# Jerx2y/Raytracer-2022

Measured on AMD Instinct MI355X. Metric: Mrays/s (primary+secondary), book-2 final scene 800x800x1000spp, higher is better.
Workload: dtype f64

## Files before the change

raytracer_2022_amd/csrc/hip/pt_device.h:

```cpp
#ifndef RT2022_PT_DEVICE_H
#define RT2022_PT_DEVICE_H

#include <hip/hip_runtime.h>
#include <stdint.h>

#include <vector>

#include "../../../include/rt2022.h"
#include "hip_owned.hpp"

namespace rt2022 {

struct MediumDev {
    double center[3], radius;
    double neg_inv_density;
    uint32_t boundary, mat;
    uint32_t sphere_boundary;
    uint32_t _pad[3];
};

struct MaterialDev {
    uint32_t tex, tex_kind;
    double albedo[3];
    double param;
// ... 27 lines not shown
    const MediumDev *media_dev;
    uint32_t media_mode;
    uint32_t n_nodes;
    uint32_t n_xforms, n_media;
    uint32_t n_spheres, n_moving_spheres;
    uint32_t n_rects;
};

struct StatsDev {
    unsigned long long paths, rays, node_visits;
    unsigned long long prim_tests[RT_KIND_COUNT];
    unsigned long long light_pdf_tests, rng_draws;
    unsigned long long op_rounds[9], op_lanes[9];
};

struct RenderArgs {
    rt_camera cam;
    uint32_t width, height, spp, max_depth;
    uint32_t n_frames, n_rows;
    uint32_t chunk, n_chunks;
    double background[3];
    double t_min;
    uint64_t seed;
    uint64_t n_pixels;
    uint64_t n_items;
    const uint32_t *row_ids;
    double *partial;
    unsigned long long *work_counter;
    double *tape;
    uint32_t ring, ring_group;
    const unsigned long long *claim_limit;
    uint32_t tuning;
    uint32_t vote_weights;
    StatsDev *stats;
    const rt_radiance_ray *rays;
};

enum SlotKind : uint32_t {
    SK_IDLE = 0,
    SK_FRESH = 1,
    SK_TRACE = 2,
    SK_MISS = 3,
    SK_LIGHT = 4,
    SK_LAMB_SOLID = 5,
    SK_LAMB_CHECKER = 6,
    SK_LAMB_NOISE = 7,
    SK_LAMB_IMAGE = 8,
    SK_METAL = 9,
    SK_DIELECTRIC = 10,
    SK_ISOTROPIC = 11,
    SK_COUNT = 12
};

constexpr uint32_t kMatKindShift = 24, kMatIndexMask = (1u << kMatKindShift) - 1u;

constexpr int kSlotsPerBlock = 4096;
constexpr uint64_t kRecBytes = 128, kRecDoubles = kRecBytes / 8, kRecWords = kRecBytes / 4;
struct WfPool {
    uint32_t n_slots;
    uint32_t n_blocks;
    uint8_t *kind;
    double *ray;
    uint32_t *hit;
    uint32_t *state;
    double *pixel_sum;
    double *tape;
    uint32_t tape_cap;
    uint16_t *list;
    uint32_t *list_n;
    uint32_t segs;
    uint32_t *next_chunk;
    uint32_t *max_list;
    uint32_t n_cus;
    uint32_t *n_active;
    uint32_t *fault;
    unsigned long long *oldest;
    uint32_t *starved_n;
    unsigned long long *dbg;
};

namespace tune {
constexpr uint32_t kSegmentsShift = 16, kClassShift = 20, kGroupsShift = 24;
constexpr uint32_t kNoNodeTable = 1u << 28, kPassTiming = 1u << 29, kLiteralStep = 1u << 30, kBoxesPlain = 1u << 31;
constexpr uint32_t quorum(uint32_t word) { return word & 0xFFu; }
constexpr uint32_t segments(uint32_t word) { return (word >> kSegmentsShift) & 0xFu; }
constexpr uint32_t class_shift(uint32_t word) { return (word >> kClassShift) & 0xFu; }
constexpr uint32_t groups(uint32_t word) { return (word >> kGroupsShift) & 0xFu; }
constexpr bool no_node_table(uint32_t word) { return (word & kNoNodeTable) != 0; }
constexpr bool pass_timing(uint32_t word) { return (word & kPassTiming) != 0; }
constexpr bool literal_step(uint32_t word) { return (word & kLiteralStep) != 0; }
constexpr bool boxes_plain(uint32_t word) { return (word >> 31) != 0; }
constexpr uint32_t for_kernels(uint32_t word, bool plain) { return (word & ~kBoxesPlain) | (plain && !literal_step(word) ? kBoxesPlain : 0u); }
constexpr uint32_t kRetiredDefault = (1u << 8) | (2u << 12);
constexpr uint32_t kDefault = 18u | kRetiredDefault | ((uint32_t)(8 * 4096 / kSlotsPerBlock > 0 ? 8 * 4096 / kSlotsPerBlock : 1) << kSegmentsShift) |
                              (2u << kClassShift) | (0u << kGroupsShift);
static_assert(kDefault == 0x00282112u, "the default tuning word");
}

constexpr int kStackSmall = 22;
constexpr int kStackMid = 30;
constexpr int kStackLarge = 64;
constexpr int kBlock = 256;
constexpr uint32_t kWfVoteWeights = 0x24444442u;
constexpr int kCacheBlock = 1024;
constexpr int kStackTiny = 16;
constexpr int kNodeCache = 1740;
constexpr int kPrimNodes = 600, kPrimSpheres = 256, kPrimMoving = 512;
constexpr int kTraceBlocksPerCU = 4;

struct QueryArgs {
    const rt_query_ray *rays;
    rt_hit *hits;
    uint64_t n_rays;
    unsigned long long *counter;
    StatsDev *stats;
};
hipError_t launch_query(const SceneDev &scene, const QueryArgs &args, uint32_t stack_need, bool counters, bool any_hit,
                        hipStream_t stream);

struct FeatureArgs {
    rt_camera cam;
    uint32_t width, height, spp, n_rows;
    double background[3];
    double t_min;
    uint64_t seed;
    uint64_t n_pixels;
    const uint32_t *row_ids;
    rt_feature *out;
    unsigned long long *counter;
    StatsDev *stats;
};
hipError_t launch_features(const SceneDev &scene, const FeatureArgs &args, uint32_t stack_need, bool counters, hipStream_t stream);

hipError_t launch_render(const SceneDev &scene, const RenderArgs &args, uint32_t stack_need, bool counters,
                         int n_blocks_hint, hipStream_t stream);
constexpr unsigned kFeatMisc = 1;
constexpr unsigned kFeatMovers = 2;
constexpr unsigned kFeatVolumes = 4;

constexpr int kMaxGroups = 8;
// ... 59 lines not shown
```

raytracer_2022_amd/csrc/hip/pt_wavefront.hip:

```cpp
#include <algorithm>
#include <cstdio>
#include <cstdlib>
#include <type_traits>
#include <vector>

#include "pt_common.hpp"

namespace rt2022 {

namespace {

constexpr int S = kSlotsPerBlock;
constexpr uint32_t kOriginClasses = 4u;
constexpr uint32_t kListBins = 16 * kOriginClasses * 8;
constexpr uint32_t kChunk = 256;
constexpr int kShadeWaves = 3;
constexpr int kLeanBlocks = 5;
constexpr int kSphereReps = 2, kNodeReps = 1, kBoxReps = 2, kMiscReps = 2;

typedef double f64x2 __attribute__((ext_vector_type(2)));
typedef double f64x2_a8 __attribute__((ext_vector_type(2), aligned(8)));
typedef uint32_t u32x4 __attribute__((ext_vector_type(4)));
typedef uint32_t u32x2 __attribute__((ext_vector_type(2)));
typedef float f32x2 __attribute__((ext_vector_type(2)));
// ... 139 lines not shown
        }
        case RT_KIND_RECT: {
            RectP rp{(uint32_t)rtm::d2u(q.r2.y), q.r0.x, q.r0.y, q.r1.x, q.r1.y, q.r2.x};
            rect_record(rp, 0u, r, t, rec);
            break;
        }
        case RT_KIND_BOX: {
            const double p0x = q.r0.x, p0y = q.r0.y, p0z = q.r1.x, p1x = q.r1.y, p1y = q.r2.x, p1z = q.r2.y;
            const uint32_t i = w.face;
            RectP rp;
            if (i < 2) rp = RectP{RT_RECT_XY, p0x, p1x, p0y, p1y, i == 0 ? p1z : p0z};
            else if (i < 4) rp = RectP{RT_RECT_XZ, p0x, p1x, p0z, p1z, i == 2 ? p1y : p0y};
            else rp = RectP{RT_RECT_YZ, p0y, p1y, p0z, p1z, i == 4 ? p1x : p0x};
            rect_record(rp, 0u, r, t, rec);
            break;
        }
        case RT_KIND_TRIANGLE: {
            const Vec3 a(q.r0.x, q.r0.y, q.r1.x), b(q.r1.y, q.r2.x, q.r2.y), c(q.r3.x, q.r3.y, q.r4.x);
            Vec3 n = rtm::to_unit(rtm::cross(b - a, c - a));
            Vec3 p = r.o + r.d * t;
            double a1 = a.x - b.x, b1 = a.x - c.x, c1 = a.x - p.x;
            double a2 = a.y - b.y, b2 = a.y - c.y, c2 = a.y - p.y;
            rec.u = (c1 * b2 - b1 * c2) / (a1 * b2 - b1 * a2);
            rec.v = (a1 * c2 - a2 * c1) / (a1 * b2 - b1 * a2);
            rec.p = p; rec.t = t;
            rec.set_face_normal(r.d, n);
            break;
        }
        case RT_KIND_RING: {
            rec.p = r.o + r.d * t; rec.t = t; rec.u = 0.0; rec.v = 0.0;
            rec.set_face_normal(r.d, Vec3(0.0, 1.0, 0.0));
            break;
        }
        default: {
            rec.p = r.o + r.d * t; rec.normal = Vec3(1.0, 0.0, 0.0); rec.t = t; rec.u = 0.0; rec.v = 0.0;
            rec.front_face = true;
            break;
        }
    }
    if (w.leaf & RT_REF_FLIP) rec.front_face = !rec.front_face;
    for (uint32_t lvl = w.chain.n; lvl > 0; lvl--) {
        XRay moved = ray_at_level(s, w.chain, lvl, world);
        xform_record(s, w.chain.at(lvl - 1), moved, rec);
    }
}
RT_DEV Vec3 texture_value_top(const SceneDev &s, uint32_t tex, uint32_t tex_kind, Vec3 color, double u, double v, Vec3 p) {
    if (tex_kind == RT_TEX_SOLID) return color;
    return texture_value(s, tex, u, v, p);
}

}

#ifdef RT2022_SHADE_PROBE
#define SP_DECL unsigned long long sp_t = wall_clock64(), sp_acc[10] = {0, 0, 0, 0, 0, 0, 0, 0, 0, 0}
#define SP_MARK(i) do { unsigned long long sp_n = wall_clock64(); sp_acc[i] += sp_n - sp_t; sp_t = sp_n; } while (0)
#define SP_FLUSH() do { if (tid == 0 && pool.dbg) for (int sp_i = 0; sp_i < 10; sp_i++) atomicAdd(&pool.dbg[64 + sp_i], sp_acc[sp_i]); } while (0)
#else
#define SP_DECL do {} while (0)
#define SP_MARK(i) do {} while (0)
#define SP_FLUSH() do {} while (0)
#endif

template <bool STATS, bool RING = false, bool RAYS = false>
__global__ void __launch_bounds__(kBlock, kShadeWaves) wf_shade(const SceneDev s, const RenderArgs *__restrict__ ap, const WfPool pool, const uint32_t parity) {
    __shared__ uint32_t hist[SK_COUNT];
    __shared__ uint32_t cursor[SK_COUNT];
    __shared__ uint32_t sorted[S];
    __shared__ uint32_t n_sorted;
    __shared__ uint8_t new_kind[S];
    __shared__ uint32_t bins[kListBins];
    __shared__ uint8_t new_oct[S];
    __shared__ uint16_t fresh_q[S];
    static_assert(kSlotsPerBlock <= 32768 && kSlotsPerBlock % kBlock == 0, "a segment's slot index shares a u16 with one flag bit (fresh_q), and the sorts deal S / kBlock slots to every thread");
    static_assert(kSlotsPerBlock <= 65536, "`sorted` packs slot | kind << 16");
    __shared__ uint32_t n_fresh;
    const RenderArgs &a = *ap;
    const PoolView pv{pool};
    const uint32_t base = blockIdx.x * (uint32_t)S;
    const uint32_t tid = threadIdx.x;
    const unsigned lane = tid & 63u;
    Counters<STATS> cnt;

    constexpr uint32_t kLdsLights = 8;
    __shared__ LightRec lights_lds[kLdsLights];
    __shared__ PrimTable prim_tab;
    prim_table_fill(s, prim_tab, tid);
    if (tid < kLdsLights && tid < s.n_lights) lights_lds[tid] = fetch_light(s, tid);
    auto light_at = [&](uint32_t li) { return li < kLdsLights ? lights_lds[li] : fetch_light(s, li); };
    SP_DECL;
    if (tid < SK_COUNT) hist[tid] = 0;
    if (tid == 0) n_fresh = 0;
    __syncthreads();
    const uint32_t n_rays = pool.list_n[blockIdx.x] < (uint32_t)S ? pool.list_n[blockIdx.x] : (uint32_t)S;
    const uint32_t n_starved_in = RING ? (pool.starved_n[blockIdx.x] < (uint32_t)S - n_rays ? pool.starved_n[blockIdx.x] : (uint32_t)S - n_rays) : 0u;
    const uint32_t n_listed = n_rays + n_starved_in;
    uint32_t my_kind[S / kBlock], my_slot[S / kBlock];
#pragma unroll
    for (int i = 0; i < S / kBlock; i++) {
        const uint32_t e = (uint32_t)(i * kBlock) + tid;
        uint32_t k = SK_IDLE, ls = 0;
        if (e < n_listed) { k = pool.kind[base + e]; ls = pool.list[base + e]; }
        my_kind[i] = k; my_slot[i] = ls;
        new_kind[e] = (uint8_t)SK_IDLE;
        if (k != SK_IDLE) atomicAdd(&hist[k], 1u);
    }
    __syncthreads();
    if (tid == 0) {
        uint32_t acc = 0;
        for (uint32_t k = 0; k < SK_COUNT; k++) { cursor[k] = acc; acc += hist[k]; }
        n_sorted = acc;
    }
    __syncthreads();
#pragma unroll
    for (int i = 0; i < S / kBlock; i++) {
        uint32_t k = my_kind[i];
        if (k != SK_IDLE) sorted[atomicAdd(&cursor[k], 1u)] = my_slot[i] | (k << 16);
    }
    __syncthreads();
    SP_MARK(0);
    const uint32_t total = n_sorted;
    const Vec3 background = ld3(a.background);
    const bool single = a.chunk == 1 && a.spp > 0 && a.max_depth > 0;
    const bool small_job = a.n_items <= 0xFFFFFFFFull;
    const uint32_t step_shift = tune::class_shift(a.tuning);

    unsigned long long my_oldest = ~0ull;
    for (uint32_t j0 = 0; j0 < total; j0 += kBlock) {
        const uint32_t j = j0 + tid;
        const bool on = j < total;
        uint32_t slot = 0, kind = SK_IDLE;
        if (on) { uint32_t e = sorted[j]; slot = base + (e & 0xFFFFu); kind = e >> 16; }
        if (on && kind == SK_TRACE) atomicOr(pool.fault, 1u);
        bool alive = false;
        bool ended = false;
        Ray r;
        Rng rng;
        Vec3 Lterm(0.0, 0.0, 0.0);
        SlotTape tape{pool.tape + (uint64_t)slot * pool.tape_cap * 4};
        SlotState stt{};
        Winner w;
        w.t = 0.0; w.leaf = 0; w.face = 0; w.chain.n = 0; w.chain.c0 = w.chain.c1 = w.chain.c2 = w.chain.c3 = 0;
        uint32_t steps = 0;
        uint32_t mat_word = 0;
        PrimRegs prim{{0.0, 0.0}, {0.0, 0.0}, {0.0, 0.0}, {0.0, 0.0}, {0.0, 0.0}};
        f64x2 md0{0.0, 0.0}, md1{0.0, 0.0}, md2{0.0, 0.0}, md3{0.0, 0.0}, md4{0.0, 0.0};
        if (on) {
            stt = load_state(pool, slot);
            if (kind > SK_MISS) {
                uint64_t rs;
                r = pv.load_ray(slot, rs);
                rng = Rng(rs);
                const u32x4 *hq = reinterpret_cast<const u32x4 *>(pool.hit + (uint64_t)slot * kRecWords);
                u32x4 ha = hq[0], hb = hq[1];
                t_pin(ha); t_pin(hb);
                bool have_mat;
                PoolView::decode_hit(ha, hb, w, steps, mat_word, have_mat);
                if (!have_mat) mat_word = leaf_material_word(s, w.leaf);
                const f64x2_a8 *pp = prim_address(prim_tab, w.leaf);
                const f64x2 *mp = reinterpret_cast<const f64x2 *>(s.materials_dev + (mat_word & kMatIndexMask));
                prim.r0 = pp[0]; prim.r1 = pp[1]; prim.r2 = pp[2]; prim.r3 = pp[3]; prim.r4 = pp[4];
                md0 = mp[0]; md1 = mp[1]; md2 = mp[2]; md3 = mp[3]; md4 = mp[4];
                t_pin(prim.r0); t_pin(prim.r1); t_pin(prim.r2); t_pin(prim.r3); t_pin(prim.r4);
                t_pin(md0); t_pin(md1); t_pin(md2); t_pin(md3); t_pin(md4);
            }
        }
        SP_MARK(1);
        const uint32_t m_tex = (uint32_t)rtm::d2u(md0.x), m_tex_kind = (uint32_t)(rtm::d2u(md0.x) >> 32);
        const Vec3 m_albedo(md0.y, md1.x, md1.y), m_tex_color(md2.y, md3.x, md3.y);
        const double m_param = md2.x;
        uint32_t depth = stt.depth & 0x7FFFFFFFu;
        uint32_t tainted = stt.depth >> 31;
        uint32_t expect = steps;

        if (on && kind >= SK_MISS) {
            if (kind == SK_MISS) {
                Lterm = background;
                ended = true;
            } else {
                bool want_uv = false;
                const bool lambertian = kind >= SK_LAMB_SOLID && kind <= SK_LAMB_IMAGE;
                if (lambertian) {
                    want_uv = kind == SK_LAMB_IMAGE || kind == SK_LAMB_CHECKER;
                } else if (kind == SK_LIGHT || kind == SK_ISOTROPIC) {
                    want_uv = m_tex_kind == RT_TEX_IMAGE || m_tex_kind == RT_TEX_CHECKER;
                }
                HitRec rec;
                winner_record_regs(s, r, w, prim, rec, want_uv);
                SP_MARK(2);
                if (kind == SK_LIGHT) {
                    Lterm = rec.front_face ? texture_value_top(s, m_tex, m_tex_kind, m_tex_color, rec.u, rec.v, rec.p) : Vec3(0.0, 0.0, 0.0);
                    ended = true;
                } else {
                    Vec3 wgt;
                    double p = 1.0;
                    Vec3 dir;
                    double tm = r.tm;
                    if (lambertian) {
                        Vec3 att = texture_value_top(s, m_tex, m_tex_kind, m_tex_color, rec.u, rec.v, rec.p);
                        rtm::Onb uvw = rtm::onb_from_w(rec.normal);
                        double cosv;
                        if (s.n_lights == 0) {
                            dir = uvw.local_vec(random_cosine_direction(rng));
                            cosv = rtm::dot(rtm::to_unit(dir), uvw.w);
                            p = cosv <= 0.0 ? 0.0 : cosv / rtm::PI;
                        } else {
                            if (rng.gen_range(0.0, 1.0) < 0.5) dir = lights_random_of(s.n_lights, light_at, rec.p, rng);
                            else dir = uvw.local_vec(random_cosine_direction(rng));
                            double lp = lights_pdf_value_of<STATS>(s.n_lights, light_at, rec.p, dir, cnt);
                            cosv = rtm::dot(rtm::to_unit(dir), uvw.w);
                            double cp = cosv <= 0.0 ? 0.0 : cosv / rtm::PI;
                            p = 0.5 * lp + 0.5 * cp;
                        }
                        double cosine = rtm::dot(rec.normal, rtm::to_unit(dir));
                        double spdf = cosine < 0.0 ? 0.0 : cosine / rtm::PI;
                        wgt = att * spdf;
                    } else if (kind == SK_METAL) {
                        Vec3 reflected = rtm::reflect(rtm::to_unit(r.dir), rec.normal);
                        dir = reflected + random_in_unit_sphere(rng) * m_param;
                        wgt = m_albedo;
                        tm = 0.0;
                    } else if (kind == SK_DIELECTRIC) {
                        double refraction_ratio = rec.front_face ? 1.0 / m_param : m_param;
                        Vec3 unit_direction = rtm::to_unit(r.dir);
                        double cos_theta = rtm::fmin_(rtm::dot(-unit_direction, rec.normal), 1.0);
                        double sin_theta = rtm::sqrt_(1.0 - cos_theta * cos_theta);
                        bool cannot_refract = refraction_ratio * sin_theta > 1.0;
                        double random_double = rng.gen_range(0.0, 1.0);
                        dir = (cannot_refract || reflectance(cos_theta, refraction_ratio) > random_double)
                                  ? rtm::reflect(unit_direction, rec.normal)
                                  : rtm::refract(unit_direction, rec.normal, refraction_ratio);
                        wgt = Vec3(1.0, 1.0, 1.0);
                    } else {
                        wgt = texture_value_top(s, m_tex, m_tex_kind, m_tex_color, rec.u, rec.v, rec.p);
                        dir = random_in_unit_sphere(rng);
                    }
                    uint32_t nb = a.max_depth - depth;
                    tape.put(nb, wgt, p);
                    tainted |= (t_finite_s(wgt.x) && t_finite_s(wgt.y) && t_finite_s(wgt.z) && p == p && p != 0.0) ? 0u : 1u;
                    r = Ray(rec.p, dir, tm);
                    depth--;
                    if (depth == 0) ended = true;
                    else alive = true;
                }
            }
            SP_MARK(3);
            if (ended) {
                uint32_t nb = a.max_depth - depth;
                Vec3 Lp(0.0, 0.0, 0.0);
                if (!(nb >= 1 && !tainted && Lterm.x == 0.0 && Lterm.y == 0.0 && Lterm.z == 0.0)) Lp = tape.unwind(nb, Lterm);
                if (single) {
                    double *o = a.partial + stt.item * 3;
                    o[0] = 0.0 + Lp.x; o[1] = 0.0 + Lp.y; o[2] = 0.0 + Lp.z;
                } else {
                    double2 *ps = reinterpret_cast<double2 *>(pool.pixel_sum + (uint64_t)slot * 4);
                    double2 s0 = ps[0], s1 = ps[1];
                    ps[0] = make_double2(s0.x + Lp.x, s0.y + Lp.y);
                    ps[1] = make_double2(s1.x + Lp.z, 0.0);
                }
            }
// ... 213 lines not shown
    constexpr uint32_t kPer = kListBins > (uint32_t)kBlock ? kListBins / (uint32_t)kBlock : 1u;
    static_assert(kPer * (uint32_t)kBlock >= kListBins, "bins per thread");
    __shared__ uint32_t wave_tot[kBlock / 64];
    {
        uint32_t v[kPer], sum = 0;
#pragma unroll
        for (uint32_t j = 0; j < kPer; j++) { const uint32_t k = tid * kPer + j; v[j] = k < kListBins ? bins[k] : 0u; sum += v[j]; }
        uint32_t inc = sum;
#pragma unroll
        for (int d = 1; d < 64; d <<= 1) { const uint32_t t = (uint32_t)__shfl_up((int)inc, d); if ((int)lane >= d) inc += t; }
        if (lane == 63) wave_tot[tid >> 6] = inc;
        __syncthreads();
        uint32_t excl = inc - sum;
        for (uint32_t wv = 0; wv < (tid >> 6); wv++) excl += wave_tot[wv];
#pragma unroll
        for (uint32_t j = 0; j < kPer; j++) { const uint32_t k = tid * kPer + j; if (k < kListBins) bins[k] = excl; excl += v[j]; }
    }
    if (tid == 0) {
        uint32_t acc = 0;
        for (int wv = 0; wv < kBlock / 64; wv++) acc += wave_tot[wv];
        pool.list_n[blockIdx.x] = acc;
        uint32_t going = acc;
        if (RING) {
            list_total = acc;
            pool.starved_n[blockIdx.x] = n_starved_out;
            going += n_starved_out;
            if (seg_oldest != ~0ull) atomicMin(&pool.oldest[parity], seg_oldest);
            if (blockIdx.x == 0) pool.oldest[parity ^ 1u] = ~0ull;
        }
        if (going) atomicAdd(&pool.n_active[parity], going);
        if (acc) atomicMax(&pool.max_list[parity], acc);
        if (blockIdx.x == 0) { pool.n_active[parity ^ 1u] = 0; pool.max_list[parity ^ 1u] = 0; *pool.next_chunk = 0; }
    }
    __syncthreads();
    if (RING) {
#pragma unroll
        for (int i = 0; i < S / kBlock; i++)
            if (my_starved[i] != 0xFFFFFFFFu) {
                const uint32_t pos = base + list_total + my_starved[i];
                pool.list[pos] = (uint16_t)((uint32_t)(i * kBlock) + tid);
                pool.kind[pos] = (uint8_t)SK_FRESH;
            }
    }
#pragma unroll
    for (int i = 0; i < S / kBlock; i++)
        if (my_key[i] < kListBins) {
            const uint32_t pos = base + atomicAdd(&bins[my_key[i]], 1u);
            pool.list[pos] = (uint16_t)((uint32_t)(i * kBlock) + tid);
            pool.kind[pos] = (uint8_t)SK_TRACE;
        }
    if (STATS) cnt.flush_wave(a.stats);
    SP_MARK(7);
    SP_FLUSH();
}

namespace {

struct TLane {
    XRay cur;
    Vec3 inv;
    double a_len;
    double tm;
    double closest;
    double t_lo;
    double sub_closest;
    double med_t1;
    uint32_t med_ref;
    Rng rng;
    Chain ctx;
    Chain win_chain;
    uint32_t win_leaf, win_face;
    uint32_t win_mat;
    double stash_ix, stash_iz;
    uint32_t stash_level;
    uint32_t near_at[3], far_at[3];
    f32x2 p32[3];
    float e_ray;
    uint32_t slot;
    uint32_t entry;
    uint32_t steps;
    int sp;
    uint32_t top, op;
    uint32_t flags;
};

template <int STACK, int WG = kBlock>
struct TStack {
    uint32_t *col;
    RT_DEV void push(TLane &L, uint32_t ref) { if (L.sp < STACK) { col[L.sp * WG] = ref; L.sp++; } }
    RT_DEV uint32_t pop(TLane &L) { if (L.sp > 0) { L.sp--; return col[L.sp * WG]; } return REF_EMPTY; }
};

constexpr uint32_t kPlain = 1u, kHasRay = 2u, kSubFound = 4u, kNeed64 = 8u;
RT_DEV void t_flag(TLane &L, uint32_t bit, bool on) { L.flags = on ? (L.flags | bit) : (L.flags & ~bit); asm volatile("" : "+v"(L.flags)); }
RT_DEV bool t_finite(double x) { return (rtm::d2u(x) & 0x7FF0000000000000ull) != 0x7FF0000000000000ull; }
RT_DEV void t_flags(TLane &L, bool boxes_plain) {
    const bool plain = boxes_plain && t_finite(L.inv.x) && t_finite(L.inv.y) && t_finite(L.inv.z) && L.inv.x != 0.0 && L.inv.y != 0.0 &&
              L.inv.z != 0.0 && t_finite(L.cur.o.x) && t_finite(L.cur.o.y) && t_finite(L.cur.o.z);
    t_flag(L, kPlain, plain);
}
RT_DEV void t_slabs(TLane &L, uint32_t table_at) {
#pragma unroll
    for (int i = 0; i < 3; i++) {
        const bool neg = L.inv[i] < 0.0;
        L.near_at[i] = table_at + (neg ? 24u : 0u) + 8u * (uint32_t)i;
        L.far_at[i] = table_at + (neg ? 0u : 24u) + 8u * (uint32_t)i;
    }
}
constexpr uint32_t kNode32Words = 11, kNode32Bytes = 4 * kNode32Words;
constexpr float kF32RelBound = 4.5f * 0x1p-24f, kF32RayBound = 6.5f * 0x1p-24f;
RT_DEV void t_slabs32(TLane &L, uint32_t table_at) {
    float e = 0.0f;
    bool ok = true;
#pragma unroll
    for (int i = 0; i < 3; i++) {
        const bool neg = L.inv[i] < 0.0;
        L.near_at[i] = table_at + 12u * (uint32_t)i + (neg ? 4u : 0u);
        const float i32 = (float)L.inv[i], n32 = (float)(-(L.cur.o[i] * L.inv[i]));
        L.p32[i] = (f32x2){i32, n32};
        e = __builtin_fmaxf(e, __builtin_fabsf(n32));
        const float ai = __builtin_fabsf(i32);
        ok = ok && ai >= 1e-30f && ai <= 1e30f;
    }
    L.e_ray = ok ? __builtin_fmaf(e, kF32RayBound, 2e-8f) : __builtin_inff();
}
RT_DEV void t_slabs32g(TLane &L) {
    float e = 0.0f;
    bool ok = true;
#pragma unroll
    for (int i = 0; i < 3; i++) {
        const float i32 = (float)L.inv[i], n32 = (float)(-(L.cur.o[i] * L.inv[i]));
        L.p32[i] = (f32x2){i32, n32};
        e = __builtin_fmaxf(e, __builtin_fabsf(n32));
        const float ai = __builtin_fabsf(i32);
        ok = ok && ai >= 1e-30f && ai <= 1e30f;
    }
    L.e_ray = ok ? __builtin_fmaf(e, kF32RayBound, 2e-8f) : __builtin_inff();
}
RT_DEV void t_set_cur(TLane &L, const XRay &c, bool boxes_plain) {
    L.cur = c;
    L.inv = Vec3(1.0 / c.d.x, 1.0 / c.d.y, 1.0 / c.d.z);
    L.a_len = c.d.length_sqr();
    t_flags(L, boxes_plain);
}
RT_DEV double t_hi(const TLane &L) { return L.med_ref ? L.sub_closest : L.closest; }
RT_DEV void t_accept(TLane &L, double t, uint32_t face, uint32_t mat_word) {
// ... 153 lines not shown
                const f64x2_a8 *qp = reinterpret_cast<const f64x2_a8 *>(s.spheres + i);
                sp_lds[2 * i] = qp[0]; sp_lds[2 * i + 1] = qp[1];
                spm_lds[i] = s.spheres[i].mat;
            }
            for (uint32_t i = tid; i < 5u * s.n_moving_spheres && i < 5u * (uint32_t)kPrimMoving; i += (uint32_t)WG)
                ms_lds[i] = reinterpret_cast<const f64x2 *>(s.moving_spheres)[i];
        }
    }
    if (kLdsXforms || kLdsMedia || CACHE > 0) {
        if (tid < 2 * kLdsXforms && tid < 2 * s.n_xforms) xf_lds[tid] = reinterpret_cast<const u32x4 *>(s.xforms)[tid];
        if (tid >= 64 && tid < 64 + 4 * kLdsMedia && tid < 64 + 4 * s.n_media) md_lds[tid - 64] = reinterpret_cast<const f64x2 *>(s.media_dev)[tid - 64];
        __syncthreads();
    }
    auto xform_words = [&](uint32_t idx, u32x4 &x0, f64x2 &x1) {
        if (kLdsXforms && idx < kLdsXforms) { x0 = xf_lds[2 * idx]; x1 = reinterpret_cast<const f64x2 *>(xf_lds)[2 * idx + 1]; }
        else { const u32x4 *xp = reinterpret_cast<const u32x4 *>(s.xforms + idx); x0 = xp[0]; x1 = reinterpret_cast<const f64x2 *>(xp)[1]; }
    };
    auto ray_at = [&](const Chain &ch, uint32_t level, XRay r) {
        for (uint32_t i = 0; i < level && i < RT_MAX_XFORM_DEPTH; i++) {
            const uint32_t ref = ch.at(i);
            u32x4 x0; f64x2 x1;
            xform_words(RT_REF_INDEX(ref), x0, x1);
            r = xform_ray_p(RT_REF_KIND(ref), rtm::u2d(((uint64_t)x0.w << 32) | x0.z), x1.x, x1.y, r);
        }
        return r;
    };
    double *const wray = wray_lds + (kStash ? tid : 0u);

    const uint32_t n_seg = pool.n_blocks;
    const uint32_t total_ids = ((pool.max_list[parity] + kChunk - 1u) / kChunk) * n_seg;
    typedef uint32_t u32x4 __attribute__((ext_vector_type(4)));
    __shared__ u32x4 chunk_lds[WG / 64];
    volatile u32x4 *const cs = &chunk_lds[tid >> 6];
    if (lane == 0) *cs = (u32x4){0u, 0u, 0u, 0u};
    const bool probe = PROBE && pool.dbg != nullptr;
    unsigned long long t_start = 0, t_dry = 0;
    bool dry_seen = false;
    if (probe) t_start = wall_clock64();

    TP_DECL;
#ifdef RT2022_F32_CENSUS
    unsigned f32_steps = 0, f32_undecided = 0, f32_wrong = 0;
#endif
    TLane L;
    L.flags = 0; L.op = OP_SHADE; L.top = REF_EMPTY; L.sp = 0; L.slot = 0; L.entry = 0; L.steps = 0;
    L.closest = rtm::F64_MAX; L.a_len = 0.0; L.tm = 0.0;
    L.t_lo = t_min; L.sub_closest = rtm::INF; L.med_t1 = 0.0; L.med_ref = 0;
    L.ctx.c0 = L.ctx.c1 = L.ctx.c2 = L.ctx.c3 = 0; L.ctx.n = 0;
    L.win_chain = L.ctx; L.win_leaf = REF_EMPTY; L.win_face = 0; L.win_mat = 0;
    L.stash_ix = 0.0; L.stash_iz = 0.0; L.stash_level = 0xFFFFFFFFu;
    const int node_quorum = (int)tune::quorum(tuning);
    constexpr int tail_factor = 2;
    const bool boxes_plain = tune::boxes_plain(tuning);
    unsigned census_rounds[9] = {0, 0, 0, 0, 0, 0, 0, 0, 0}, census_lanes[9] = {0, 0, 0, 0, 0, 0, 0, 0, 0};
    unsigned long long ctab = kClassifyTable;
    uint32_t ref_empty = REF_EMPTY;
    asm volatile("" : "+s"(ctab), "+v"(ref_empty));
    constexpr bool kSlabs = CACHE > 0 && !PARTIAL && !(FEAT & kFeatMisc) && !kF32;
    typedef const __attribute__((address_space(3))) f64x2 *LdsBoxPtr;
    typedef const __attribute__((address_space(3))) u32x2 *LdsRefPtr;
    LdsBoxPtr ncb = (LdsBoxPtr)nc_box;
    LdsRefPtr ncr = (LdsRefPtr)nc_ref;
    if (CACHE > 0) asm volatile("" : "+v"(ncb), "+v"(ncr));
    uint32_t table32_at = (uint32_t)(uintptr_t)(const __attribute__((address_space(3))) uint32_t *)nc32;
    if (kF32) asm volatile("" : "+v"(table32_at));
    const uint32_t table_at = kF32 ? table32_at : (uint32_t)(uintptr_t)ncb;
    L.near_at[0] = L.near_at[1] = L.near_at[2] = L.far_at[0] = L.far_at[1] = L.far_at[2] = table_at;
    L.p32[0] = L.p32[1] = L.p32[2] = (f32x2){0.0f, 0.0f}; L.e_ray = __builtin_inff();
    uint32_t refs32_at = table32_at + 36u;
    if (kF32) asm volatile("" : "+v"(refs32_at));

    for (;;) {
        {
            bool isn = (kF32 || kF32G) ? (L.op | ((L.flags ^ kPlain) & (kPlain | kNeed64))) == 0u : (L.op | (~L.flags & kPlain)) == 0u;
            int nn = __popcll(wballot(isn));
            const int pending = __popcll(wballot(L.op != OP_IDLE));
            const int tail_threshold = tail_factor * pending / (tail_factor + 1) + 1;
            const int threshold = node_quorum < tail_threshold ? node_quorum : tail_threshold;
            double tlo_c = L.t_lo, thi_c = t_hi(L);
            asm volatile("" : "+v"(tlo_c), "+v"(thi_c));
            const bool entered = isn && nn >= threshold;
            float tlo32 = 0.0f, thi32 = 0.0f;
            if ((kF32 || kF32G) && entered) {
                tlo32 = (float)tlo_c; thi32 = (float)thi_c;
                asm volatile("" : "+v"(tlo32), "+v"(thi32));
            }
            if (entered) do {
                if (STATS) { const unsigned long long am = wballot(true); if ((int)lane == __ffsll((long long)am) - 1) { census_rounds[8]++; census_lanes[8] += (unsigned)nn; } }
                {
                const uint32_t nidx = RT_REF_INDEX(L.top);
                const int below_sp = L.sp > 0 ? L.sp - 1 : 0;
                double bmin[3], bmax[3];
                uint32_t left, right, below;
                bool hit, undecided = false;
                if (kF32) {
                    uint32_t a0, a1, a2, ar;
                    asm("v_mad_u32_u24 %0, %1, 44, %2" : "=v"(a0) : "v"(L.top), "v"(L.near_at[0]));
                    asm("v_mad_u32_u24 %0, %1, 44, %2" : "=v"(a1) : "v"(L.top), "v"(L.near_at[1]));
                    asm("v_mad_u32_u24 %0, %1, 44, %2" : "=v"(a2) : "v"(L.top), "v"(L.near_at[2]));
                    asm("v_mad_u32_u24 %0, %1, 44, %2" : "=v"(ar) : "v"(L.top), "v"(refs32_at));
                    static_assert(kNode32Bytes == 44, "the multiply-adds above carry the record size");
                    const uint32_t below_at = (uint32_t)(uintptr_t)(__attribute__((address_space(3))) uint32_t *)(st.col + below_sp * WG);
                    f32x2 bx, by, bz, tx, ty, tz;
                    u32x2 cr;
                    asm volatile("ds_read2_b32 %0, %5 offset1:1\n\tds_read2_b32 %1, %6 offset1:1\n\tds_read2_b32 %2, %7 offset1:1\n\t"
                                 "ds_read2_b32 %3, %8 offset1:1\n\tds_read_b32 %4, %9\n\ts_waitcnt lgkmcnt(0)"
// ... 388 lines not shown
                if (kSlabs) t_slabs(L, table_at); if (kF32) t_slabs32(L, table_at); if (kF32G) t_slabs32g(L);
                T_SETTLE();
            } else {
                uint32_t kind = RT_REF_KIND(L.top), idx = RT_REF_INDEX(L.top);
                if (kind == RT_KIND_LIST) {
                    cnt.prim(kind);
                    const rt_list &l = s.lists[idx];
                    for (uint32_t i = l.count; i > 0; i--) st.push(L, s.list_items[l.first + i - 1]);
                    T_NEXT();
                } else if (L.ctx.n < RT_MAX_XFORM_DEPTH) {
#pragma unroll 1
                    for (uint32_t rep = 0; rep < RT_MAX_XFORM_DEPTH; rep++) {
                        cnt.prim(kind);
                        u32x4 x0;
                        f64x2 x1;
                        xform_words(idx, x0, x1);
                        t_pin(x0); t_pin(x1);
                        const double p0 = rtm::u2d(((uint64_t)x0.w << 32) | x0.z), p1 = x1.x, p2 = x1.y;
                        if (kind == RT_KIND_TRANSLATE) {
                            L.cur.o = L.cur.o - Vec3(p0, p1, p2);
                        } else if (kind == RT_KIND_ROTATE_Y) {
                            const double ox = p1 * L.cur.o.x - p0 * L.cur.o.z, oz = p0 * L.cur.o.x + p1 * L.cur.o.z;
                            const double dx = p1 * L.cur.d.x - p0 * L.cur.d.z, dz = p0 * L.cur.d.x + p1 * L.cur.d.z;
                            L.cur.o.x = ox; L.cur.o.z = oz; L.cur.d.x = dx; L.cur.d.z = dz;
                            if (kStashInv) { L.stash_ix = L.inv.x; L.stash_iz = L.inv.z; L.stash_level = L.ctx.n; }
                            L.inv.x = 1.0 / dx; L.inv.z = 1.0 / dz;
                            L.a_len = L.cur.d.length_sqr();
                        } else {
                            L.cur.o = L.cur.o / p0;
                        }
                        L.ctx.push(L.top);
                        st.push(L, REF_POPCTX);
                        L.top = x0.y;
                        kind = RT_REF_KIND(L.top); idx = RT_REF_INDEX(L.top);
                        if (!(kind >= RT_KIND_TRANSLATE && kind <= RT_KIND_ZOOM && L.ctx.n < RT_MAX_XFORM_DEPTH)) break;
                    }
                    t_flags(L, boxes_plain);
                    if (kSlabs) t_slabs(L, table_at); if (kF32) t_slabs32(L, table_at); if (kF32G) t_slabs32g(L);
                    T_SETTLE();
                } else {
                    cnt.prim(kind);
                    T_NEXT();
                }
            }
        } else if (best == OP_SHADE) {
            if (L.flags & kHasRay) {
                uint32_t slot = L.slot;
                bool found = L.win_leaf != REF_EMPTY;
                uint32_t kind = SK_MISS;
                const uint32_t steps16 = (L.steps > 0xFFFFu ? 0xFFFFu : L.steps) << 16;
                if (found) {
                    pv.store_hit(slot, L.closest, L.win_leaf, L.win_face | (L.win_chain.n << 4) | steps16, L.win_chain, L.win_mat);
                    kind = L.win_mat >> kMatKindShift;
                }
                pool.kind[L.entry] = (uint8_t)kind;
                if (L.rng.draws) { pv.store_rng(slot, L.rng.s); cnt.draws(L.rng.draws); }
                t_flag(L, kHasRay, false);
            }
            const unsigned long long m = wballot(true);
            const int leader = __ffsll((long long)m) - 1;
            uint32_t need = (uint32_t)__popcll(m);
            uint32_t rank = (uint32_t)__popcll(m & ((1ull << lane) - 1ull));
            uint32_t entry_idx = 0xFFFFFFFFu;
            const u32x4 cs_now = *cs;
            uint32_t ch_base = cs_now.x, ch_n = cs_now.y, ch_taken = cs_now.z;
            bool drained = cs_now.w != 0;
            for (;;) {
                const uint32_t avail = ch_n - ch_taken;
                if (entry_idx == 0xFFFFFFFFu) {
                    if (rank < avail) entry_idx = ch_base + ch_taken + rank;
                    else rank -= avail;
                }
                const uint32_t take = need < avail ? need : avail;
                ch_taken += take;
                need -= take;
                if (need == 0 || drained) break;
                uint32_t id = 0;
                if ((int)lane == leader) id = atomicAdd(pool.next_chunk, 1u);
                id = (uint32_t)__shfl((int)id, leader);
                if (id >= total_ids) { drained = true; break; }
                const uint32_t slice = id / n_seg, seg = id - slice * n_seg, first = slice * kChunk;
                const uint32_t n = pool.list_n[seg];
                ch_n = n > first ? (n - first < kChunk ? n - first : kChunk) : 0u;
                ch_base = seg * (uint32_t)S + first;
                ch_taken = 0;
            }
            if ((int)lane == leader) *cs = (u32x4){ch_base, ch_n, ch_taken, drained ? 1u : 0u};
            if (probe && !dry_seen && drained) { dry_seen = true; t_dry = wall_clock64(); }
            if (entry_idx != 0xFFFFFFFFu) {
                const uint32_t sbase = entry_idx & ~((uint32_t)S - 1u);
                L.entry = entry_idx;
                L.slot = sbase + pool.list[entry_idx];
                uint64_t rs;
                Ray wr = pv.load_ray(L.slot, rs);
                L.tm = wr.tm;
                L.rng = Rng(rs);
                t_set_cur(L, XRay{wr.orig, wr.dir}, boxes_plain);
                if (kSlabs) t_slabs(L, table_at); if (kF32) t_slabs32(L, table_at); if (kF32G) t_slabs32g(L);
                if (FEAT & kFeatMovers) L.stash_level = 0xFFFFFFFFu;
                if (kStash) {
                    wray[0 * WG] = wr.orig.x; wray[1 * WG] = wr.orig.y; wray[2 * WG] = wr.orig.z;
                    wray[3 * WG] = wr.dir.x; wray[4 * WG] = wr.dir.y; wray[5 * WG] = wr.dir.z;
                }
                L.closest = rtm::F64_MAX;
                L.steps = 0;
                L.t_lo = t_min; L.med_ref = 0;
                L.win_leaf = REF_EMPTY; L.win_face = 0;
                L.ctx.n = 0;
                L.sp = 0;
                L.top = s.root;
                T_SETTLE();
                t_flag(L, kHasRay, true);
            } else {
                L.op = OP_IDLE;
            }
        }
        TP_MARK(2 + best);
    }
    TP_FLUSH();
#ifdef RT2022_F32_CENSUS
    if (f32_steps) atomicAdd(&g_f32_census[0], (unsigned long long)f32_steps);
    if (f32_undecided) atomicAdd(&g_f32_census[1], (unsigned long long)f32_undecided);
    if (f32_wrong) atomicAdd(&g_f32_census[2], (unsigned long long)f32_wrong);
#endif
    if (probe && lane == 0) {
        unsigned long long t_end = wall_clock64();
        atomicMin(&pool.dbg[0], t_start);
        atomicMax(&pool.dbg[1], t_end);
        atomicAdd(&pool.dbg[2], t_end - t_start);
        atomicAdd(&pool.dbg[3], t_end - (dry_seen ? t_dry : t_end));
        atomicAdd(&pool.dbg[4], 1ull);
        if (tid == 0) { pool.dbg[8 + 2 * blockIdx.x] = t_start; pool.dbg[9 + 2 * blockIdx.x] = t_end; }
    }
    if (STATS) {
        cnt.flush_wave(stats);
        if (stats)
            for (int o = 0; o < 9; o++) {
                if (census_rounds[o]) atomicAdd(&stats->op_rounds[o], (unsigned long long)census_rounds[o]);
                if (census_lanes[o]) atomicAdd(&stats->op_lanes[o], (unsigned long long)census_lanes[o]);
            }
    }
}

__global__ void __launch_bounds__(256) wf_init(uint8_t *kind, uint16_t *list, uint32_t *list_n, uint32_t n_slots, uint32_t used) {
    uint32_t i = blockIdx.x * blockDim.x + threadIdx.x;
    if (i < n_slots) {
        const uint32_t local = i % (uint32_t)S;
        kind[i] = local < used ? (uint8_t)SK_FRESH : (uint8_t)SK_IDLE;
        list[i] = (uint16_t)local;
// ... 343 lines not shown
    }
    return hipSuccess;
}
}

hipError_t f32_slab_census(unsigned long long out[5]) {
    unsigned long long c[3] = {0, 0, 0};
    hipError_t e = hipMemcpyFromSymbol(c, HIP_SYMBOL(g_f32_census), sizeof(c));
    if (e != hipSuccess) return e;
    const unsigned long long zero[3] = {0, 0, 0};
    e = hipMemcpyToSymbol(HIP_SYMBOL(g_f32_census), zero, sizeof(zero));
    out[0] = c[0]; out[1] = c[1]; out[4] = c[2];
#ifdef RT2022_F32_CENSUS
    out[2] = 1; out[3] = 2;
#else
    out[2] = 0; out[3] = 1;
#endif
    return e;
}

void trace_variant(const SceneDev &scene, uint32_t stack_need, uint32_t tuning, unsigned features, uint32_t out[4]) {
    const TraceChoice c = choose_trace(scene, stack_need, tuning, features, false, false);
    const bool table = c.table != kTablePlain;
    const bool f32 = table ? f32_lds(c.feat, true, c.table == kTablePartial, c.table == kTablePrims, c.spheres)
                           : f32_hbm(c.feat, false, false, c.spheres, c.stats, c.probe);
    out[0] = (uint32_t)(table ? kCacheBlock : kBlock);
    out[1] = (uint32_t)c.stack;
    out[2] = !table ? 0u : scene.n_nodes < (uint32_t)kNodeCache ? scene.n_nodes : (uint32_t)kNodeCache;
    out[3] = (c.table == kTablePrims ? 1u : 0u) | (f32 ? 2u : 0u);
}

#ifdef RT2022_TRACE_PROBE
static void print_trace_probe(const WfPool &pool) {
    unsigned long long h[12];
    if (hipMemcpy(h, pool.dbg + 96, sizeof h, hipMemcpyDeviceToHost) == hipSuccess) {
        static const char *const names[12] = {"node_fast", "vote", "node", "sphere", "rect", "box", "medium", "misc", "ctx", "done", "rest", "-"};
        double tot = 0; for (int i = 0; i < 11; i++) tot += (double)h[i];
        fprintf(stderr, "trace probe (shader-clock ticks of all waves and passes; share):");
        for (int i = 0; i < 11; i++) fprintf(stderr, " %s %.3f", names[i], tot > 0 ? (double)h[i] / tot : 0.0);
        fprintf(stderr, "  total %.3e ticks\n", tot);
    }
    (void)hipMemset(pool.dbg + 96, 0, 12 * sizeof(unsigned long long));
}
#endif
#ifdef RT2022_SHADE_PROBE
static void print_shade_probe(const WfPool &pool) {
    unsigned long long h[10];
    if (hipMemcpy(h, pool.dbg + 64, sizeof h, hipMemcpyDeviceToHost) == hipSuccess) {
        double tot = 0; for (int i = 0; i < 8; i++) tot += (double)h[i];
        fprintf(stderr, "shade probe (ticks of wave 0, all workgroups and passes; share):");
        for (int i = 0; i < 8; i++) fprintf(stderr, " [%d] %.3f", i, tot > 0 ? (double)h[i] / tot : 0.0);
        fprintf(stderr, "  total %.3e ticks\n", tot);
    }
    (void)hipMemset(pool.dbg + 64, 0, 10 * sizeof(unsigned long long));
}
#endif

hipError_t launch_render_wavefront(WfRender &r) {
    const auto drain = [&r] {
        for (int g = 0; g < kMaxGroups; g++)
            if (r.gs->stream[g]) (void)hipStreamSynchronize(r.gs->stream[g]);
        (void)hipStreamSynchronize(r.stream);
    };
    hipError_t e;
    try { e = PassDriver(r).run(); } catch (...) { drain(); throw; }
    if (e != hipSuccess) { drain(); return e; }
#ifdef RT2022_TRACE_PROBE
    if (r.pool->dbg) print_trace_probe(*r.pool);
#endif
#ifdef RT2022_SHADE_PROBE
    if (r.pool->dbg) print_shade_probe(*r.pool);
#endif
    return hipMemcpy(&r.fault, r.pool->fault, sizeof r.fault, hipMemcpyDeviceToHost);
}

}
```

Measured before the change: 3201.

## Sort shade queue by primitive class and predicted light-sampling coin

The trace kernel now writes a sub-key next to the material kind in each slot's kind byte. The sub-key holds the winning primitive class (box/rect, static sphere, moved sphere) and a pre-drawn bit predicting whether a Lambertian bounce will sample the lights. The shade kernel's counting sort goes from 12 bins to 128 kind×sub-key bins, with the prefix sum done as a single-wave scan, so lanes that share a record-construction path and light-sampling branch sit in the same wave. The aim is to cut divergence in shade, in exchange for more histogram bins, extra hashing in trace, and a coin prediction that may not match the actual draw. Probe census counters are added for measurement.

```diff
diff --git a/raytracer_2022_amd/csrc/hip/pt_device.h b/raytracer_2022_amd/csrc/hip/pt_device.h
--- a/raytracer_2022_amd/csrc/hip/pt_device.h
+++ b/raytracer_2022_amd/csrc/hip/pt_device.h
@@ -103,6 +103,12 @@
     SK_COUNT = 12
 };
 
+constexpr uint32_t kKindMask = 0xFu, kSubShift = 4, kSubKeys = 8, kKeyMask = 0x7Fu;
+constexpr uint32_t kSubBox = 1u, kSubSphere = 2u, kSubSphereMoved = 3u, kSubCoin = 4u;
+constexpr uint32_t kSortBins = 16u * kSubKeys;
+static_assert(SK_COUNT <= kKindMask + 1u && (kKindMask + 1u) * kSubKeys == kKeyMask + 1u, "kind and sub-key share the low seven bits of the byte");
+constexpr uint32_t sort_bin(uint32_t key) { return (key & kKindMask) * kSubKeys + ((key & kKeyMask) >> kSubShift); }
+
 constexpr uint32_t kMatKindShift = 24, kMatIndexMask = (1u << kMatKindShift) - 1u;
 
 constexpr int kSlotsPerBlock = 4096;
@@ -132,11 +138,13 @@
 
 namespace tune {
 constexpr uint32_t kSegmentsShift = 16, kClassShift = 20, kGroupsShift = 24;
+constexpr uint32_t kNoSubKey = 1u << 15;
 constexpr uint32_t kNoNodeTable = 1u << 28, kPassTiming = 1u << 29, kLiteralStep = 1u << 30, kBoxesPlain = 1u << 31;
 constexpr uint32_t quorum(uint32_t word) { return word & 0xFFu; }
 constexpr uint32_t segments(uint32_t word) { return (word >> kSegmentsShift) & 0xFu; }
 constexpr uint32_t class_shift(uint32_t word) { return (word >> kClassShift) & 0xFu; }
 constexpr uint32_t groups(uint32_t word) { return (word >> kGroupsShift) & 0xFu; }
+constexpr bool no_sub_key(uint32_t word) { return (word & kNoSubKey) != 0; }
 constexpr bool no_node_table(uint32_t word) { return (word & kNoNodeTable) != 0; }
 constexpr bool pass_timing(uint32_t word) { return (word & kPassTiming) != 0; }
 constexpr bool literal_step(uint32_t word) { return (word & kLiteralStep) != 0; }
diff --git a/raytracer_2022_amd/csrc/hip/pt_wavefront.hip b/raytracer_2022_amd/csrc/hip/pt_wavefront.hip
--- a/raytracer_2022_amd/csrc/hip/pt_wavefront.hip
+++ b/raytracer_2022_amd/csrc/hip/pt_wavefront.hip
@@ -215,6 +215,24 @@
 }
 
 #ifdef RT2022_SHADE_PROBE
+#define SP_CENSUS_DECL unsigned long long sp_cn[8] = {0, 0, 0, 0, 0, 0, 0, 0}; const bool sp_keys = !tune::no_sub_key(ap->tuning)
+#define SP_LEADER(m) ((int)(threadIdx.x & 63u) == __ffsll((long long)(m)) - 1)
+#define SP_TURN(on, kind) do { const unsigned long long sp_m = wballot(on); if (sp_m) { \
+        const uint32_t sp_k0 = (uint32_t)__shfl((int)(kind), __ffsll((long long)sp_m) - 1); const bool sp_mixed = wballot((on) && (kind) != sp_k0) != 0; \
+        if (SP_LEADER(sp_m)) { sp_cn[0]++; sp_cn[1] += sp_mixed ? 1u : 0u; } } } while (0)
+#define SP_ARMS(arm, first, last, at) do { const unsigned long long sp_all = wballot(true); \
+        for (uint32_t sp_a = (first); sp_a <= (last); sp_a++) { const unsigned long long sp_m = wballot((arm) == sp_a); \
+            if (sp_m && SP_LEADER(sp_all)) { sp_cn[at]++; sp_cn[(at) + 1] += (unsigned long long)__popcll(sp_m); } } } while (0)
+#define SP_RECORD(key, w) do { const uint32_t sp_lk = RT_REF_KIND((w).leaf); \
+        const uint32_t sp_cls = (sp_lk == RT_KIND_SPHERE || sp_lk == RT_KIND_MOVING_SPHERE) ? ((w).chain.n ? kSubSphereMoved : kSubSphere) : (sp_lk == RT_KIND_RECT || sp_lk == RT_KIND_BOX) ? kSubBox : 0u; \
+        SP_ARMS(sp_cls, 0u, 3u, 2); if (sp_keys && (((key) >> kSubShift) & 3u) != sp_cls) sp_cn[6]++; } while (0)
+#define SP_SCATTER(kind, coin_known, state) do { \
+        const uint32_t sp_arm = 2u * (kind) + (((coin_known) && (rtm::mix64((state) + 0x9E3779B97F4A7C15ull) >> 63)) ? 1u : 0u); \
+        SP_ARMS(sp_arm, 2u * SK_LIGHT, 2u * SK_COUNT - 1u, 4); } while (0)
+#define SP_COIN(key, to_lights) do { if (sp_keys && ((((key) >> kSubShift) & kSubCoin) != 0) == (to_lights)) sp_cn[7]++; } while (0)
+#define SP_CENSUS_FLUSH() do { for (int sp_i = 0; sp_i < 8; sp_i++) { unsigned long long sp_v = sp_cn[sp_i]; \
+        for (int sp_d = 32; sp_d > 0; sp_d >>= 1) sp_v += __shfl_xor(sp_v, sp_d); \
+        if ((threadIdx.x & 63u) == 0 && sp_v && pool.dbg) atomicAdd(&pool.dbg[80 + sp_i], sp_v); } } while (0)
 #define SP_DECL unsigned long long sp_t = wall_clock64(), sp_acc[10] = {0, 0, 0, 0, 0, 0, 0, 0, 0, 0}
 #define SP_MARK(i) do { unsigned long long sp_n = wall_clock64(); sp_acc[i] += sp_n - sp_t; sp_t = sp_n; } while (0)
 #define SP_FLUSH() do { if (tid == 0 && pool.dbg) for (int sp_i = 0; sp_i < 10; sp_i++) atomicAdd(&pool.dbg[64 + sp_i], sp_acc[sp_i]); } while (0)
@@ -222,12 +240,18 @@
 #define SP_DECL do {} while (0)
 #define SP_MARK(i) do {} while (0)
 #define SP_FLUSH() do {} while (0)
+#define SP_CENSUS_DECL do {} while (0)
+#define SP_TURN(on, kind) do {} while (0)
+#define SP_RECORD(key, w) do {} while (0)
+#define SP_SCATTER(kind, coin_known, state) do {} while (0)
+#define SP_COIN(key, to_lights) do {} while (0)
+#define SP_CENSUS_FLUSH() do {} while (0)
 #endif
 
 template <bool STATS, bool RING = false, bool RAYS = false>
 __global__ void __launch_bounds__(kBlock, kShadeWaves) wf_shade(const SceneDev s, const RenderArgs *__restrict__ ap, const WfPool pool, const uint32_t parity) {
-    __shared__ uint32_t hist[SK_COUNT];
-    __shared__ uint32_t cursor[SK_COUNT];
+    __shared__ uint32_t hist[kSortBins];
+    __shared__ uint32_t cursor[kSortBins];
     __shared__ uint32_t sorted[S];
     __shared__ uint32_t n_sorted;
     __shared__ uint8_t new_kind[S];
@@ -235,7 +259,8 @@
     __shared__ uint8_t new_oct[S];
     __shared__ uint16_t fresh_q[S];
     static_assert(kSlotsPerBlock <= 32768 && kSlotsPerBlock % kBlock == 0, "a segment's slot index shares a u16 with one flag bit (fresh_q), and the sorts deal S / kBlock slots to every thread");
-    static_assert(kSlotsPerBlock <= 65536, "`sorted` packs slot | kind << 16");
+    static_assert(kSlotsPerBlock <= 65536 && kKeyMask <= 0xFFFFu, "`sorted` packs slot | (kind | sub-key << kSubShift) << 16");
+    static_assert(kSortBins == 128 && kSortBins <= (uint32_t)kBlock, "the bins' prefix sums are one wave's scan, two bins per lane");
     __shared__ uint32_t n_fresh;
     const RenderArgs &a = *ap;
     const PoolView pv{pool};
@@ -251,33 +276,39 @@
     if (tid < kLdsLights && tid < s.n_lights) lights_lds[tid] = fetch_light(s, tid);
     auto light_at = [&](uint32_t li) { return li < kLdsLights ? lights_lds[li] : fetch_light(s, li); };
     SP_DECL;
-    if (tid < SK_COUNT) hist[tid] = 0;
+    SP_CENSUS_DECL;
+    if (tid < kSortBins) hist[tid] = 0;
     if (tid == 0) n_fresh = 0;
     __syncthreads();
     const uint32_t n_rays = pool.list_n[blockIdx.x] < (uint32_t)S ? pool.list_n[blockIdx.x] : (uint32_t)S;
     const uint32_t n_starved_in = RING ? (pool.starved_n[blockIdx.x] < (uint32_t)S - n_rays ? pool.starved_n[blockIdx.x] : (uint32_t)S - n_rays) : 0u;
     const uint32_t n_listed = n_rays + n_starved_in;
+    const uint32_t key_mask = tune::no_sub_key(a.tuning) ? kKindMask : kKeyMask;
     uint32_t my_kind[S / kBlock], my_slot[S / kBlock];
 #pragma unroll
     for (int i = 0; i < S / kBlock; i++) {
         const uint32_t e = (uint32_t)(i * kBlock) + tid;
         uint32_t k = SK_IDLE, ls = 0;
-        if (e < n_listed) { k = pool.kind[base + e]; ls = pool.list[base + e]; }
+        if (e < n_listed) { k = pool.kind[base + e] & key_mask; ls = pool.list[base + e]; }
         my_kind[i] = k; my_slot[i] = ls;
         new_kind[e] = (uint8_t)SK_IDLE;
-        if (k != SK_IDLE) atomicAdd(&hist[k], 1u);
+        if ((k & kKindMask) != SK_IDLE) atomicAdd(&hist[sort_bin(k)], 1u);
     }
     __syncthreads();
-    if (tid == 0) {
-        uint32_t acc = 0;
-        for (uint32_t k = 0; k < SK_COUNT; k++) { cursor[k] = acc; acc += hist[k]; }
-        n_sorted = acc;
+    if (tid < 64) {
+        const uint32_t c0 = hist[2 * tid], c1 = hist[2 * tid + 1];
+        uint32_t inc = c0 + c1;
+#pragma unroll
+        for (int d = 1; d < 64; d <<= 1) { const uint32_t t = (uint32_t)__shfl_up((int)inc, d); if ((int)lane >= d) inc += t; }
+        const uint32_t excl = inc - (c0 + c1);
+        cursor[2 * tid] = excl; cursor[2 * tid + 1] = excl + c0;
+        if (tid == 63) n_sorted = inc;
     }
     __syncthreads();
 #pragma unroll
     for (int i = 0; i < S / kBlock; i++) {
         uint32_t k = my_kind[i];
-        if (k != SK_IDLE) sorted[atomicAdd(&cursor[k], 1u)] = my_slot[i] | (k << 16);
+        if ((k & kKindMask) != SK_IDLE) sorted[atomicAdd(&cursor[sort_bin(k)], 1u)] = my_slot[i] | (k << 16);
     }
     __syncthreads();
     SP_MARK(0);
@@ -292,7 +323,9 @@
         const uint32_t j = j0 + tid;
         const bool on = j < total;
         uint32_t slot = 0, kind = SK_IDLE;
-        if (on) { uint32_t e = sorted[j]; slot = base + (e & 0xFFFFu); kind = e >> 16; }
+        uint32_t sort_key = SK_IDLE;
+        if (on) { uint32_t e = sorted[j]; slot = base + (e & 0xFFFFu); sort_key = e >> 16; kind = sort_key & kKindMask; }
+        SP_TURN(on, kind);
         if (on && kind == SK_TRACE) atomicOr(pool.fault, 1u);
         bool alive = false;
         bool ended = false;
@@ -348,8 +381,10 @@
                     want_uv = m_tex_kind == RT_TEX_IMAGE || m_tex_kind == RT_TEX_CHECKER;
                 }
                 HitRec rec;
+                SP_RECORD(sort_key, w);
                 winner_record_regs(s, r, w, prim, rec, want_uv);
                 SP_MARK(2);
+                SP_SCATTER(kind, lambertian && s.n_lights != 0, rng.s);
                 if (kind == SK_LIGHT) {
                     Lterm = rec.front_face ? texture_value_top(s, m_tex, m_tex_kind, m_tex_color, rec.u, rec.v, rec.p) : Vec3(0.0, 0.0, 0.0);
                     ended = true;
@@ -367,7 +402,9 @@
                             cosv = rtm::dot(rtm::to_unit(dir), uvw.w);
                             p = cosv <= 0.0 ? 0.0 : cosv / rtm::PI;
                         } else {
-                            if (rng.gen_range(0.0, 1.0) < 0.5) dir = lights_random_of(s.n_lights, light_at, rec.p, rng);
+                            const bool to_lights = rng.gen_range(0.0, 1.0) < 0.5;
+                            SP_COIN(sort_key, to_lights);
+                            if (to_lights) dir = lights_random_of(s.n_lights, light_at, rec.p, rng);
                             else dir = uvw.local_vec(random_cosine_direction(rng));
                             double lp = lights_pdf_value_of<STATS>(s.n_lights, light_at, rec.p, dir, cnt);
                             cosv = rtm::dot(rtm::to_unit(dir), uvw.w);
@@ -687,6 +724,7 @@
     if (STATS) cnt.flush_wave(a.stats);
     SP_MARK(7);
     SP_FLUSH();
+    SP_CENSUS_FLUSH();
 }
 
 namespace {
@@ -726,7 +764,7 @@
     RT_DEV uint32_t pop(TLane &L) { if (L.sp > 0) { L.sp--; return col[L.sp * WG]; } return REF_EMPTY; }
 };
 
-constexpr uint32_t kPlain = 1u, kHasRay = 2u, kSubFound = 4u, kNeed64 = 8u;
+constexpr uint32_t kPlain = 1u, kHasRay = 2u, kSubFound = 4u, kNeed64 = 8u, kCoin = 16u;
 RT_DEV void t_flag(TLane &L, uint32_t bit, bool on) { L.flags = on ? (L.flags | bit) : (L.flags & ~bit); asm volatile("" : "+v"(L.flags)); }
 RT_DEV bool t_finite(double x) { return (rtm::d2u(x) & 0x7FF0000000000000ull) != 0x7FF0000000000000ull; }
 RT_DEV void t_flags(TLane &L, bool boxes_plain) {
@@ -986,6 +1024,7 @@
     const int node_quorum = (int)tune::quorum(tuning);
     constexpr int tail_factor = 2;
     const bool boxes_plain = tune::boxes_plain(tuning);
+    const bool sub_keys = !tune::no_sub_key(tuning), coin_keys = s.n_lights != 0;
     unsigned census_rounds[9] = {0, 0, 0, 0, 0, 0, 0, 0, 0}, census_lanes[9] = {0, 0, 0, 0, 0, 0, 0, 0, 0};
     unsigned long long ctab = kClassifyTable;
     uint32_t ref_empty = REF_EMPTY;
@@ -1480,6 +1519,14 @@
                 if (found) {
                     pv.store_hit(slot, L.closest, L.win_leaf, L.win_face | (L.win_chain.n << 4) | steps16, L.win_chain, L.win_mat);
                     kind = L.win_mat >> kMatKindShift;
+                    if (sub_keys) {
+                        const uint32_t lk = RT_REF_KIND(L.win_leaf);
+                        uint32_t sub = (lk == RT_KIND_SPHERE || lk == RT_KIND_MOVING_SPHERE) ? (L.win_chain.n ? kSubSphereMoved : kSubSphere)
+                                     : (lk == RT_KIND_RECT || lk == RT_KIND_BOX) ? kSubBox : 0u;
+                        const bool heads = (FEAT & kFeatVolumes) ? (coin_keys && (rtm::mix64(L.rng.s + 0x9E3779B97F4A7C15ull) >> 63) != 0) : (L.flags & kCoin) != 0;
+                        const bool coin = heads && kind >= SK_LAMB_SOLID && kind <= SK_LAMB_IMAGE;
+                        kind |= (sub | (coin ? kSubCoin : 0u)) << kSubShift;
+                    }
                 }
                 pool.kind[L.entry] = (uint8_t)kind;
                 if (L.rng.draws) { pv.store_rng(slot, L.rng.s); cnt.draws(L.rng.draws); }
@@ -1523,6 +1570,7 @@
                 Ray wr = pv.load_ray(L.slot, rs);
                 L.tm = wr.tm;
                 L.rng = Rng(rs);
+                if (!(FEAT & kFeatVolumes)) t_flag(L, kCoin, sub_keys && coin_keys && (rtm::mix64(rs + 0x9E3779B97F4A7C15ull) >> 63) != 0);
                 t_set_cur(L, XRay{wr.orig, wr.dir}, boxes_plain);
                 if (kSlabs) t_slabs(L, table_at); if (kF32) t_slabs32(L, table_at); if (kF32G) t_slabs32g(L);
                 if (FEAT & kFeatMovers) L.stash_level = 0xFFFFFFFFu;
@@ -1972,7 +2020,14 @@
         for (int i = 0; i < 8; i++) fprintf(stderr, " [%d] %.3f", i, tot > 0 ? (double)h[i] / tot : 0.0);
         fprintf(stderr, "  total %.3e ticks\n", tot);
     }
-    (void)hipMemset(pool.dbg + 64, 0, 10 * sizeof(unsigned long long));
+    unsigned long long c[8];
+    if (hipMemcpy(c, pool.dbg + 80, sizeof c, hipMemcpyDeviceToHost) == hipSuccess) {
+        const auto util = [](unsigned long long lanes, unsigned long long arms) { return arms ? (double)lanes / (64.0 * (double)arms) : 0.0; };
+        fprintf(stderr, "shade census (all waves and passes): wave turns %llu, mixed kinds %llu (%.3f); section 2: %llu record arms, %llu lanes, utilisation %.3f; "
+                        "section 3: %llu arms, %llu lanes, utilisation %.3f; sorted against their sub-key: record class %llu, coin %llu\n",
+                c[0], c[1], c[0] ? (double)c[1] / (double)c[0] : 0.0, c[2], c[3], util(c[3], c[2]), c[4], c[5], util(c[5], c[4]), c[6], c[7]);
+    }
+    (void)hipMemset(pool.dbg + 64, 0, 24 * sizeof(unsigned long long));
 }
 #endif
 
```

Measured after the change: 3198. No clear change (-0.1%).
